# NVIDIA-AI-IOT/redtail

Hardware: AMD Instinct MI355X
Metric: stereo pairs/sec, ResNet18-2D 1257x369 (higher is better)
Workload: dtype f32

## Files before the change

### redtail_amd/csrc/kernels/conv_split.hip.h

```cpp
#pragma once
#include <type_traits>
#include "common.hip.h"
#include "conv_mfma.hip.h"

namespace rt {

constexpr float kSplitScale = 2048.f;
constexpr float kSplitInv = 1.f / 2048.f;

struct S3Split {
    f16x4 hi, lo;
};
__device__ static __forceinline__ S3Split s3_split(f32x4 v) {
    S3Split s;
#ifdef HIPEMU
#pragma unroll
    for (int j = 0; j < 4; j++) {
        const _Float16 h = (_Float16)v[j];
        s.hi[j] = h;
        s.lo[j] = (_Float16)((v[j] - (float)h) * kSplitScale);
    }
#else
    unsigned h[2], l[2];
#pragma unroll
// ... 198 lines not shown
        RT_TSTAMP();
    }
#ifdef RT_KERNEL_TIMING
    __builtin_amdgcn_s_waitcnt(0);
    if (dbgp && tid == 0) { dbgp[14] = __builtin_amdgcn_s_memtime(); dbgp[15] = __builtin_amdgcn_s_memrealtime() - rt0; }
#endif
}

}

namespace rt {

template <int KH, int KW, int S, int NW_ = 4>
struct S3Cfg {
    static constexpr int NW = NW_, TY = NW_, TX = 32, CC = 16, TAPS = KH * KW, NT = 64 * NW_;
    static constexpr int PR = (TY - 1) * S + KH, PC = (TX - 1) * S + KW;
    static constexpr int PCH = (PC + 1) / 2;
    static constexpr int PCL = S == 2 ? 2 * PCH : PC;
    static constexpr int NPART = NW / 4;
    static constexpr int NPIX = PR * PC, NKP = ((NPIX + NPART - 1) / NPART + 63) / 64;
    static constexpr int PXB = 80;
    static constexpr int W_SLOTS = TAPS * 2 * 2 * 32;
    static constexpr int NK_W = (W_SLOTS + NT - 1) / NT;
    static constexpr int IN_BYTES = PR * PCL * PXB, GRP_BYTES = IN_BYTES + W_SLOTS * 16;
    static constexpr int KS_MAX = NW_ != 4 ? 1 : (S == 2 ? 2 : 4);
    static constexpr int max_groups(int want) {
        int ks = want < 1 ? 1 : (want > KS_MAX ? KS_MAX : want);
        while (ks > 1 && (ks == 3 || ks * GRP_BYTES < (ks - 1) * NW * 64 * 16 * 4)) ks--;
        return ks;
    }
    static_assert(IN_BYTES % 16 == 0, "weight image alignment");
    static_assert(S == 1 || S == 2, "stride 1 or 2");
};

#ifndef RT_S3_WAVES
#define RT_S3_WAVES(S) ((S) == 2 ? 2 : 4)
#endif
template <int KH, int KW, int S, bool XIL, bool YIL, int NW = 4, typename TIN = float, typename TOUT = float>
__global__ void __launch_bounds__(64 * NW * (S3Cfg<KH, KW, S, NW>::KS_MAX)) RT_WAVES_PER_EU(RT_S3_WAVES(S)) conv_s3_kernel(ConvArgs p) {
    using Cfg = S3Cfg<KH, KW, S, NW>;
    constexpr bool XF16 = std::is_same<TIN, _Float16>::value, YF16 = std::is_same<TOUT, _Float16>::value;
    constexpr unsigned ESX = Io<TIN>::ES, ESY = Io<TOUT>::ES;
    static_assert(!XIL || !XF16, "interleaved fp16 input: conv_f16mma_kernel");
    constexpr int TY = Cfg::TY, TX = Cfg::TX, CC = Cfg::CC, TAPS = Cfg::TAPS, PC = Cfg::PC, PCL = Cfg::PCL, PXB = Cfg::PXB;
    constexpr int NKP = Cfg::NKP, NK_W = Cfg::NK_W, NT = Cfg::NT;

    constexpr int IN_BYTES = Cfg::IN_BYTES, GRP_BYTES = Cfg::GRP_BYTES;
#ifdef HIPEMU
    HIP_DYNAMIC_SHARED(char, smem)
#else
    extern __shared__ __attribute__((aligned(16))) char smem[];
#endif

    const int tid_wg = threadIdx.x;
    const int KS = Cfg::KS_MAX == 1 ? 1 : __builtin_amdgcn_readfirstlane((int)blockDim.x / NT);
    const int kgi = Cfg::KS_MAX == 1 ? 0 : __builtin_amdgcn_readfirstlane(tid_wg / NT);
    const int tid = tid_wg - kgi * NT;
    char* const sIn = smem + kgi * GRP_BYTES;
    f32x4* const sW = reinterpret_cast<f32x4*>(smem + kgi * GRP_BYTES + IN_BYTES);
#ifdef RT_KERNEL_TIMING
    unsigned long long* dbgp = (p.dbg && kgi == 0) ? p.dbg + ((size_t)(blockIdx.z * gridDim.y + blockIdx.y) * gridDim.x + blockIdx.x) * 16 : nullptr;
    int dbi = 0;
    const unsigned long long rt0 = __builtin_amdgcn_s_memrealtime();
#endif
    RT_TSTAMP();
    const int lane = tid & 63;
    const int kg = lane >> 5, l31 = lane & 31;
    const int wv = __builtin_amdgcn_readfirstlane(tid >> 6);

    RT_WG_TILE_NB(p, tile, zi, n, nblk)
    const int tx0 = (tile % p.tiles_x) * TX;
    const int ty0 = (tile / p.tiles_x) * TY;
    const char* __restrict__ xb = elem_ptr(p.x, (int64_t)n * p.x_bstride, ESX);
    const int nchunks = p.CinPad / CC;
    int pad_y = p.pad_y, pad_x = p.pad_x, Ho = p.Ho, Wo = p.Wo, ch_row = zi;
    int64_t y_off = p.y_off + (int64_t)zi * p.y_zstride, w_off = 0, r_off = y_off, r_off_il8 = y_off;
    int64_t y_off_il4 = 4 * p.y_off + (int64_t)zi * p.y_zstride, r_off_il4 = y_off_il4;
    unsigned tap_mask = ~0u;
    if (p.zs) {
        const ZSlice z = p.zs[zi];
        pad_y = z.pad_y; pad_x = z.pad_x; Ho = z.Ho; Wo = z.Wo; ch_row = z.ch_row; y_off = z.y_off; w_off = z.w_off;
        r_off = z.r_off; r_off_il8 = z.r_off_il8;
        y_off_il4 = 4 * z.y_off;
        r_off_il4 = z.r_off_il4;
        tap_mask = z.tap_mask;
    }
    const int act = p.act;

    const int sg = wv & 3, spart = wv >> 2;
    const int* __restrict__ tab = p.ch_off + (int64_t)ch_row * p.CinPad + 4 * sg;
    unsigned voff[NKP];
    int lidx[NKP], xcol[NKP];
    const int* __restrict__ shtab = p.ch_shift ? p.ch_shift + (int64_t)ch_row * p.CinPad + 4 * sg : nullptr;
#pragma unroll
    for (int k = 0; k < NKP; k++) {
        const int pidx = spart * (NKP * 64) + lane + 64 * k;
        const int pr = pidx / PC, pc = pidx - pr * PC;
        const int iy = ty0 * S - pad_y + pr, ix = tx0 * S - pad_x + pc;
        const bool own = pidx < Cfg::NPIX && lane + 64 * k < NKP * 64;
        xcol[k] = ix;
        voff[k] = (own && iy >= 0 && iy < p.Hi && ix >= 0 && ix < p.Wi) ? (unsigned)(iy * p.x_pitch + ix) * (XIL ? 16u : ESX) : kBufOOB;
        const int col = S == 2 ? (pc & 1) * Cfg::PCH + (pc >> 1) : pc;
        lidx[k] = own ? (pr * PCL + col) * PXB + sg * 8 : -1;
    }
    const char* __restrict__ wsrc = reinterpret_cast<const char*>(p.w) + (w_off + ((int64_t)nblk * nchunks) * Cfg::W_SLOTS) * 16;
    const buf_rsrc rs_w = make_buf(wsrc);

    f32x4 rin[NKP];
    f32x4 rw[NK_W];
    auto prefetch = [&](int ch) {
        if constexpr (XIL) {
            const int off = tab[ch * CC];
            const int sh = shtab ? shtab[ch * CC] : 0;
            const buf_rsrc rs = make_buf(xb, off >= 0);
#pragma unroll
            for (int k = 0; k < NKP; k++) {
                const unsigned vo = sh == 0 ? voff[k] : ((voff[k] != kBufOOB && xcol[k] >= sh) ? voff[k] - (unsigned)sh * 16u : kBufOOB);
                rin[k] = buf_load4(rs, vo, (unsigned)off * 4u);
            }
        } else {
            const int sh = shtab ? shtab[ch * CC] : 0;
#pragma unroll
            for (int j = 0; j < 4; j++) {
                const int off = tab[ch * CC + j];
                const buf_rsrc rs = make_buf(xb, off >= 0);
#pragma unroll
                for (int k = 0; k < NKP; k++) {
                    const unsigned vo = sh == 0 ? voff[k] : ((voff[k] != kBufOOB && xcol[k] >= sh) ? voff[k] - (unsigned)sh * ESX : kBufOOB);
                    rin[k][j] = Io<TIN>::load(rs, vo, (unsigned)off * ESX);
                }
            }
        }
        const unsigned so = (unsigned)ch * (unsigned)(Cfg::W_SLOTS * 16);
#pragma unroll
        for (int k = 0; k < NK_W; k++) {
            const int idx = tid + NT * k;
            rw[k] = buf_load4(rs_w, idx < Cfg::W_SLOTS ? (unsigned)idx * 16u : kBufOOB, so);
        }
    };
    auto stage_to_lds = [&]() {
#pragma unroll
        for (int k = 0; k < NKP; k++) {
            if (lidx[k] < 0) continue;
            if constexpr (XF16) {
                f16x4 h;
#pragma unroll
                for (int j = 0; j < 4; j++) h[j] = (_Float16)rin[k][j];
                *reinterpret_cast<f16x4*>(sIn + lidx[k]) = h;
            } else {
                const S3Split s = s3_split(rin[k]);
                *reinterpret_cast<f16x4*>(sIn + lidx[k]) = s.hi;
                *reinterpret_cast<f16x4*>(sIn + lidx[k] + 32) = s.lo;
            }
        }
#pragma unroll
        for (int k = 0; k < NK_W; k++) {
            const int idx = tid + NT * k;
            if (idx < Cfg::W_SLOTS) sW[idx] = rw[k];
        }
    };

    const int64_t ybase = (int64_t)n * p.y_bstride + y_off;
    const int64_t rbase = (int64_t)n * p.r_bstride + r_off;
    const int cs32 = (int)p.y_cstride, rs32 = (int)p.r_cstride;
    const int oy = ty0 + wv, ox = tx0 + l31;
    const bool inb = oy < Ho && ox < Wo;
    const bool r_il = p.r_il8 != 0;
    const int cb = nblk * 32;
    f32x4 rr[4];
    if (p.resid != nullptr && kgi == 0) {
        const buf_rsrc rs_r = make_buf(elem_ptr(p.resid, r_il ? (int64_t)n * p.r_bstride + (YF16 ? r_off_il8 : r_off_il4) : rbase, ESY));
        if (r_il && YF16) {
            const unsigned vo = inb ? (unsigned)((oy * p.y_ystride + ox * p.y_xstride) * 8 + 4 * kg) * 2u : kBufOOB;
#pragma unroll
            for (int q = 0; q < 4; q++) {
                const u32x2_t u = __builtin_amdgcn_raw_buffer_load_b64(rs_r, (cb + 8 * q + 4 * kg < p.Cout) ? vo : kBufOOB, (unsigned)((cb + 8 * q) * rs32) * 2u, 0);
#pragma unroll
                for (int e = 0; e < 4; e++) rr[q][e] = (float)__builtin_bit_cast(_Float16, (unsigned short)(u[e >> 1] >> (16 * (e & 1))));
            }
        } else if (r_il) {
            const unsigned vo = inb ? (unsigned)((oy * p.y_ystride + ox * p.y_xstride) * 4 + 4 * kg * rs32) * 4u : kBufOOB;
#pragma unroll
            for (int q = 0; q < 4; q++) rr[q] = buf_load4(rs_r, (cb + 8 * q + 4 * kg < p.Cout) ? vo : kBufOOB, (unsigned)((cb + 8 * q) * rs32) * 4u);
        } else {
            const unsigned vo = inb ? (unsigned)(oy * p.y_ystride + ox * p.y_xstride + 4 * kg * rs32) * ESY : kBufOOB;
#pragma unroll
            for (int q = 0; q < 4; q++)
#pragma unroll
                for (int e = 0; e < 4; e++)
                    rr[q][e] = Io<TOUT>::load(rs_r, (cb + 8 * q + 4 * kg + e < p.Cout) ? vo : kBufOOB, (unsigned)((cb + 8 * q + e) * rs32) * ESY);
        }
    } else {
#pragma unroll
        for (int q = 0; q < 4; q++) rr[q] = f32x4{0.f, 0.f, 0.f, 0.f};
    }

    f32x16 acc_m, acc_c;
#pragma unroll
    for (int r = 0; r < 16; r++) { acc_m[r] = 0.f; acc_c[r] = 0.f; }
    const int a_off = kg * 32 + l31;
    const bool w_exact = p.w_exact != 0;
    const int b_off = (wv * S * PCL + l31) * PXB + kg * 16;
    auto compute = [&]() {
#pragma unroll
        for (int t = 0; t < TAPS; t++) {
            if (!((tap_mask >> t) & 1u)) continue;
            const int r = t / KW, s = t % KW;
            const int col = S == 2 ? (s & 1) * Cfg::PCH + (s >> 1) : s;
            const char* bp = sIn + b_off + (r * PCL + col) * PXB;
            const f16x8 bh = *reinterpret_cast<const f16x8*>(bp);
            const f16x8 ah = __builtin_bit_cast(f16x8, sW[a_off + (t * 2 + 0) * 64]);
            acc_m = __builtin_amdgcn_mfma_f32_32x32x16_f16(ah, bh, acc_m, 0, 0, 0);
            if (!w_exact) {
                const f16x8 al = __builtin_bit_cast(f16x8, sW[a_off + (t * 2 + 1) * 64]);
                acc_c = __builtin_amdgcn_mfma_f32_32x32x16_f16(al, bh, acc_c, 0, 0, 0);
            }
            if constexpr (!XF16) {
                const f16x8 bl = *reinterpret_cast<const f16x8*>(bp + 32);
                acc_c = __builtin_amdgcn_mfma_f32_32x32x16_f16(ah, bl, acc_c, 0, 0, 0);
            }
        }
    };

    if (kgi < nchunks) prefetch(kgi);
    RT_TSTAMP();
    for (int ch = kgi; ch < nchunks + kgi; ch += KS) {
        const bool mine = KS == 1 || ch < nchunks;
        if (ch != kgi) __syncthreads();
        if (mine) stage_to_lds();
        __syncthreads();
        RT_TSTAMP();
        if (ch + KS < nchunks) prefetch(ch + KS);
        if (mine) compute();
        RT_TSTAMP();
    }

#pragma unroll
    for (int r = 0; r < 16; r++) acc_m[r] = fmaf(acc_c[r], kSplitInv, acc_m[r]);
    if (KS > 1) {
        f32x4* const red = reinterpret_cast<f32x4*>(smem);
        __syncthreads();
        if (kgi > 0) {
#pragma unroll
            for (int q = 0; q < 4; q++)
                red[(((kgi - 1) * NW + wv) * 4 + q) * 64 + lane] = f32x4{acc_m[4 * q], acc_m[4 * q + 1], acc_m[4 * q + 2], acc_m[4 * q + 3]};
        }
        __syncthreads();
        if (kgi > 0) return;
        for (int g = 1; g < KS; g++)
#pragma unroll
            for (int q = 0; q < 4; q++) {
                const f32x4 v = red[(((g - 1) * NW + wv) * 4 + q) * 64 + lane];
#pragma unroll
                for (int e = 0; e < 4; e++) acc_m[4 * q + e] += v[e];
            }
    }

    const buf_rsrc rs_y = make_buf(elem_ptr(p.y, (YIL && !YF16) ? (int64_t)n * p.y_bstride + y_off_il4 : ybase, ESY));
    auto epilogue = [&](auto ACT) {
#pragma unroll
        for (int q = 0; q < 4; q++) {
            const f32x4 bv = *reinterpret_cast<const f32x4*>(p.bias + cb + 8 * q + 4 * kg);
            f32x4 o;
#pragma unroll
            for (int e = 0; e < 4; e++)
                o[e] = apply_act_fast(acc_m[4 * q + e] + (bv[e] + rr[q][e]), decltype(ACT)::value);
            if constexpr (YIL && YF16) {
                const unsigned vo = (inb && cb + 8 * q + 4 * kg < p.Cout) ? (unsigned)((oy * p.y_ystride + ox * p.y_xstride) * 8 + 4 * kg) * 2u : kBufOOB;
                u32x2_t w2;
#pragma unroll
                for (int e = 0; e < 2; e++)
                    w2[e] = (unsigned)__builtin_bit_cast(unsigned short, (_Float16)o[2 * e]) | ((unsigned)__builtin_bit_cast(unsigned short, (_Float16)o[2 * e + 1]) << 16);
                __builtin_amdgcn_raw_buffer_store_b64(w2, rs_y, vo, (unsigned)((cb + 8 * q) * cs32) * 2u, 0);
            } else if constexpr (YIL) {
                const unsigned vo = (inb && cb + 8 * q + 4 * kg < p.Cout) ? (unsigned)((oy * p.y_ystride + ox * p.y_xstride) * 4 + 4 * kg * cs32) * 4u : kBufOOB;
                buf_store4(o, rs_y, vo, (unsigned)((cb + 8 * q) * cs32) * 4u);
            } else {
                const unsigned vo = inb ? (unsigned)(oy * p.y_ystride + ox * p.y_xstride + 4 * kg * cs32) * ESY : kBufOOB;
#pragma unroll
                for (int e = 0; e < 4; e++)
                    Io<TOUT>::store(o[e], rs_y, (cb + 8 * q + 4 * kg + e < p.Cout) ? vo : kBufOOB, (unsigned)((cb + 8 * q + e) * cs32) * ESY);
            }
        }
    };
    if (act == 1) epilogue(std::integral_constant<int, 1>{});
    else if (act == 2) epilogue(std::integral_constant<int, 2>{});
    else epilogue(std::integral_constant<int, 0>{});
    RT_TSTAMP();
#ifdef RT_KERNEL_TIMING
    __builtin_amdgcn_s_waitcnt(0);
    if (dbgp && tid == 0) { dbgp[14] = __builtin_amdgcn_s_memtime(); dbgp[15] = __builtin_amdgcn_s_memrealtime() - rt0; }
#endif
}

}

namespace rt {

struct S3FirstCfg {
    static constexpr int KH = 5, KW = 5, S = 2, TY = 4, TX = 32, CMAX = 3;
    static constexpr int PR = (TY - 1) * S + KH, PC = (TX - 1) * S + KW;
    static constexpr int NPAIR = (PC + 1) / 2;
    static constexpr int RS = 208;
    static constexpr int NTASK = CMAX * PR * NPAIR, NK = (NTASK + 255) / 256;
    static constexpr int W_SLOTS = KH * 2 * 2 * 32;
};

template <bool YIL>
__global__ void __launch_bounds__(256) RT_WAVES_PER_EU(4) conv_s3_first_kernel(ConvArgs p) {
    using Cfg = S3FirstCfg;
    constexpr int KH = Cfg::KH, S = Cfg::S, TY = Cfg::TY, TX = Cfg::TX, PR = Cfg::PR, NPAIR = Cfg::NPAIR, RS = Cfg::RS;

    __shared__ __attribute__((aligned(16))) _Float16 sHi[PR * RS];
    __shared__ __attribute__((aligned(16))) _Float16 sLo[PR * RS];

    const int tid = threadIdx.x;
    const int lane = tid & 63;
    const int kg = lane >> 5, l31 = lane & 31;
    const int wv = __builtin_amdgcn_readfirstlane(tid >> 6);

    int tile = blockIdx.x;
    if (p.xcd_order) {
        const int nwg = gridDim.x, q = nwg >> 3, r = nwg & 7;
        const int xcd = blockIdx.x & 7, idx = blockIdx.x >> 3;
        tile = (xcd < r ? xcd * (q + 1) : r * (q + 1) + (xcd - r) * q) + idx;
    }
    const int tx0 = (tile % p.tiles_x) * TX;
    const int ty0 = (tile / p.tiles_x) * TY;
    const int nblk = blockIdx.y;
    const int n = blockIdx.z;

    f32x4 wa[KH][2];
    {
        const buf_rsrc rs_w = make_buf(reinterpret_cast<const char*>(p.w) + (int64_t)nblk * Cfg::W_SLOTS * 16);
#pragma unroll
        for (int r = 0; r < KH; r++)
#pragma unroll
            for (int part = 0; part < 2; part++) wa[r][part] = buf_load4(rs_w, (unsigned)(((r * 2 + part) * 2 + kg) * 32 + l31) * 16u, 0);
    }

    const buf_rsrc rs_x = make_buf((p.x2 && n >= p.x2_from) ? p.x2 + (int64_t)(n - p.x2_from) * p.x_bstride : p.x + (int64_t)n * p.x_bstride);
    const int ix0 = tx0 * S - p.pad_x, iy0 = ty0 * S - p.pad_y;
    const int cin = p.cin_real;
#pragma unroll
    for (int k = 0; k < Cfg::NK; k++) {
        const int t = tid + 256 * k;
        const int c = t / (PR * NPAIR), rem = t - c * (PR * NPAIR);
        const int pr = rem / NPAIR, pc = 2 * (rem - pr * NPAIR);
        const int iy = iy0 + pr, ix = ix0 + pc;
        const bool own = t < Cfg::NTASK && c < cin;
        const bool row_ok = own && iy >= 0 && iy < p.Hi;
        const bool ok0 = row_ok && ix >= 0 && ix < p.Wi, ok1 = row_ok && ix + 1 >= 0 && ix + 1 < p.Wi && pc + 1 < Cfg::PC;
        const unsigned vo = (unsigned)((c * p.Hi + iy) * p.x_pitch + ix) * 4u;
        const float v0 = buf_load(rs_x, ok0 ? vo : kBufOOB, 0);
        const float v1 = buf_load(rs_x, ok1 ? vo + 4u : kBufOOB, 0);
        if (t < Cfg::NTASK) {
            const _Float16 h0 = (_Float16)v0, h1 = (_Float16)v1;
            const int o = pr * RS + pc * Cfg::CMAX + c;
            sHi[o] = h0;
            sHi[o + Cfg::CMAX] = h1;
            sLo[o] = (_Float16)((v0 - (float)h0) * kSplitScale);
            sLo[o + Cfg::CMAX] = (_Float16)((v1 - (float)h1) * kSplitScale);
        }
    }
    __syncthreads();

    f32x16 acc_m, acc_c;
#pragma unroll
    for (int r = 0; r < 16; r++) { acc_m[r] = 0.f; acc_c[r] = 0.f; }
    const unsigned* __restrict__ hi32 = reinterpret_cast<const unsigned*>(sHi);
    const unsigned* __restrict__ lo32 = reinterpret_cast<const unsigned*>(sLo);
#pragma unroll
    for (int r = 0; r < KH; r++) {
        const int base = ((wv * S + r) * RS + 6 * l31 + 8 * kg) >> 1;
        u32x4_t bh, bl;
#pragma unroll
        for (int e = 0; e < 4; e++) { bh[e] = hi32[base + e]; bl[e] = lo32[base + e]; }
        const f16x8 ah = __builtin_bit_cast(f16x8, wa[r][0]), al = __builtin_bit_cast(f16x8, wa[r][1]);
        acc_m = __builtin_amdgcn_mfma_f32_32x32x16_f16(ah, __builtin_bit_cast(f16x8, bh), acc_m, 0, 0, 0);
        acc_c = __builtin_amdgcn_mfma_f32_32x32x16_f16(al, __builtin_bit_cast(f16x8, bh), acc_c, 0, 0, 0);
        acc_c = __builtin_amdgcn_mfma_f32_32x32x16_f16(ah, __builtin_bit_cast(f16x8, bl), acc_c, 0, 0, 0);
    }

    const int oy = ty0 + wv, ox = tx0 + l31;
    const bool inb = oy < p.Ho && ox < p.Wo;
    const int cs32 = (int)p.y_cstride;
    const int cb = nblk * 32;
    const buf_rsrc rs_y = make_buf(elem_ptr(p.y, (int64_t)n * p.y_bstride + p.y_off, 4));
    const int act = p.act;
    auto epilogue = [&](auto ACT) {
#pragma unroll
        for (int q = 0; q < 4; q++) {
            const f32x4 bv = *reinterpret_cast<const f32x4*>(p.bias + cb + 8 * q + 4 * kg);
            f32x4 o;
#pragma unroll
            for (int e = 0; e < 4; e++) o[e] = apply_act_fast(fmaf(acc_c[4 * q + e], kSplitInv, acc_m[4 * q + e]) + bv[e], decltype(ACT)::value);
            if constexpr (YIL) {
                const unsigned vo = (inb && cb + 8 * q + 4 * kg < p.Cout) ? (unsigned)((oy * p.y_ystride + ox) * 4 + 4 * kg * cs32) * 4u : kBufOOB;
                buf_store4(o, rs_y, vo, (unsigned)((cb + 8 * q) * cs32) * 4u);
            } else {
                const unsigned vo = inb ? (unsigned)(oy * p.y_ystride + ox * p.y_xstride + 4 * kg * cs32) * 4u : kBufOOB;
#pragma unroll
                for (int e = 0; e < 4; e++)
                    buf_store(o[e], rs_y, (cb + 8 * q + 4 * kg + e < p.Cout) ? vo : kBufOOB, (unsigned)((cb + 8 * q + e) * cs32) * 4u);
            }
        }
    };
    if (act == 1) epilogue(std::integral_constant<int, 1>{});
    else if (act == 2) epilogue(std::integral_constant<int, 2>{});
    else epilogue(std::integral_constant<int, 0>{});
}

}

namespace rt {

struct S3RBCfg {
    static constexpr int NW = 4, TY = 4, TX = 32, NT = 256;
    static constexpr int XR = TY + 4, XC = TX + 4, XPIX = XR * XC;
    static constexpr int TR = TY + 2, TC = TX + 2, TPIX = TR * TC;
    static constexpr int TSEG = (TPIX + 31) / 32;
    static constexpr int SEGW = (TSEG + NW - 1) / NW;
    static constexpr int PXB = 80;
    static constexpr int NSLOT = XPIX * 4, NKX = (NSLOT + NT - 1) / NT;
    static constexpr int W_SLOTS = 9 * 2 * 2 * 32, NK_W = (W_SLOTS + NT - 1) / NT;
};

struct RBArgs {
    ConvArgs c;
    const float* w1;
    const float* bias1;
    int act1;
    int cmid;
    int seg;
};

template <bool XIL, bool YIL>
__global__ void __launch_bounds__(256) RT_WAVES_PER_EU(2) conv_s3rb_kernel(RBArgs a) {
    using Cfg = S3RBCfg;
    const ConvArgs& p = a.c;
    constexpr int TY = Cfg::TY, TX = Cfg::TX, XC = Cfg::XC, TC = Cfg::TC, PXB = Cfg::PXB, NT = Cfg::NT;
    constexpr int NKX = Cfg::NKX, NK_W = Cfg::NK_W, SEGW = Cfg::SEGW;

    __shared__ __attribute__((aligned(16))) f32x4 sW[Cfg::W_SLOTS];
    __shared__ __attribute__((aligned(16))) char sX[Cfg::XPIX * PXB];
    __shared__ __attribute__((aligned(16))) char sT[2][Cfg::TSEG * 32 * PXB];

    const int tid = threadIdx.x;
#ifdef RT_KERNEL_TIMING
    unsigned long long* dbgp = p.dbg ? p.dbg + ((size_t)blockIdx.z * gridDim.x + blockIdx.x) * 16 : nullptr;
    int dbi = 0;
    const unsigned long long rt0 = __builtin_amdgcn_s_memrealtime();
#endif
    RT_TSTAMP();
    const int lane = tid & 63;
    const int kg = lane >> 5, l31 = lane & 31;
    const int wv = __builtin_amdgcn_readfirstlane(tid >> 6);

    int tile = blockIdx.x;
    if (p.xcd_order) {
        const int nwg = gridDim.x, q = nwg >> 3, r = nwg & 7;
        const int xcd = blockIdx.x & 7, idx = blockIdx.x >> 3;
        tile = (xcd < r ? xcd * (q + 1) : r * (q + 1) + (xcd - r) * q) + idx;
    }
    const int tx0 = (tile % p.tiles_x) * TX;
    const int ty0 = (tile / p.tiles_x) * TY;
    const int n = blockIdx.z;
    const int H = p.Hi, W = p.Wi;

    const buf_rsrc rs_x = make_buf(elem_ptr(p.x, (int64_t)n * p.x_bstride, 4));
    const unsigned cs_x = (unsigned)p.x_cstride;
    unsigned xoff[NKX];
    int xg[NKX], xlds[NKX];
#pragma unroll
    for (int k = 0; k < NKX; k++) {
        const int idx = tid + NT * k;
        const int g = idx / Cfg::XPIX, pix = idx - g * Cfg::XPIX;
        const int pr = pix / XC, pc = pix - pr * XC;
        const int iy = ty0 - 2 + pr, ix = tx0 - 2 + pc;
        const bool in = idx < Cfg::NSLOT && iy >= 0 && iy < H && ix >= 0 && ix < W;
        xoff[k] = in ? (unsigned)(iy * p.x_pitch + ix) * (XIL ? 16u : 4u) : kBufOOB;
        xg[k] = g;
        xlds[k] = idx < Cfg::NSLOT ? pix * PXB + g * 8 : -1;
    }
    f32x4 rin[NKX];
    f32x4 rw[NK_W];
    auto gather_x = [&](int ch) {
#pragma unroll
        for (int k = 0; k < NKX; k++) {
            const int c0 = 16 * ch + 4 * xg[k];
            const bool ok = xoff[k] != kBufOOB && c0 < p.cin_real;
            if constexpr (XIL) {
                rin[k] = buf_load4(rs_x, ok ? (unsigned)c0 * cs_x * 4u + xoff[k] : kBufOOB, 0u);
            } else {
#pragma unroll
                for (int j = 0; j < 4; j++)
                    rin[k][j] = buf_load(rs_x, (ok && c0 + j < p.cin_real) ? (unsigned)(c0 + j) * cs_x * 4u + xoff[k] : kBufOOB, 0u);
            }
        }
    };
    auto gather_w = [&](const float* w, int ch) {
        const buf_rsrc rs_w = make_buf(w);
#pragma unroll
        for (int k = 0; k < NK_W; k++) {
            const int idx = tid + NT * k;
            rw[k] = buf_load4(rs_w, idx < Cfg::W_SLOTS ? (unsigned)idx * 16u : kBufOOB, (unsigned)ch * (unsigned)(Cfg::W_SLOTS * 16));
        }
    };
    auto stage_x = [&]() {
#pragma unroll
        for (int k = 0; k < NKX; k++) {
            if (xlds[k] < 0) continue;
            const S3Split s = s3_split(rin[k]);
            *reinterpret_cast<f16x4*>(sX + xlds[k]) = s.hi;
            *reinterpret_cast<f16x4*>(sX + xlds[k] + 32) = s.lo;
        }
    };
    auto stage_w = [&]() {
#pragma unroll
        for (int k = 0; k < NK_W; k++) {
            const int idx = tid + NT * k;
            if (idx < Cfg::W_SLOTS) sW[idx] = rw[k];
        }
    };
    const int a_off = kg * 32 + l31;
    auto contract = [&](const char* bp0, int row_pitch, f32x16& acc_m, f32x16& acc_c) {
#pragma unroll
        for (int t = 0; t < 9; t++) {
            const int r = t / 3, s = t % 3;
            const char* bp = bp0 + (r * row_pitch + s) * PXB;
            const f16x8 bh = *reinterpret_cast<const f16x8*>(bp);
            const f16x8 bl = *reinterpret_cast<const f16x8*>(bp + 32);
            const f16x8 ah = __builtin_bit_cast(f16x8, sW[a_off + (t * 2 + 0) * 64]);
            const f16x8 al = __builtin_bit_cast(f16x8, sW[a_off + (t * 2 + 1) * 64]);
            acc_m = __builtin_amdgcn_mfma_f32_32x32x16_f16(ah, bh, acc_m, 0, 0, 0);
            acc_c = __builtin_amdgcn_mfma_f32_32x32x16_f16(al, bh, acc_c, 0, 0, 0);
            acc_c = __builtin_amdgcn_mfma_f32_32x32x16_f16(ah, bl, acc_c, 0, 0, 0);
        }
    };

    int pt[SEGW], bx[SEGW];
#pragma unroll
    for (int i = 0; i < SEGW; i++) {
        pt[i] = (wv + Cfg::NW * i) * 32 + l31;
        const int tr = pt[i] / TC, tc = pt[i] - tr * TC;
        bx[i] = (pt[i] < Cfg::TPIX ? (tr * XC + tc) * PXB : 0) + kg * 16;
    }
    f32x16 am[SEGW], ac[SEGW];
#pragma unroll
    for (int i = 0; i < SEGW; i++)
#pragma unroll
        for (int r = 0; r < 16; r++) { am[i][r] = 0.f; ac[i][r] = 0.f; }
    const bool seg1 = wv + Cfg::NW < Cfg::TSEG;

    gather_x(0);
    gather_w(a.w1, 0);
    RT_TSTAMP();
#pragma unroll
    for (int ch = 0; ch < 2; ch++) {
        if (ch) __syncthreads();
        stage_x();
        stage_w();
        __syncthreads();
        RT_TSTAMP();
        if (ch == 0) { gather_x(1); gather_w(a.w1, 1); }
        else gather_w(p.w, 0);
        contract(sX + bx[0], XC, am[0], ac[0]);
        if (seg1) contract(sX + bx[1], XC, am[1], ac[1]);
        RT_TSTAMP();
    }
#pragma unroll
    for (int i = 0; i < SEGW; i++) {
        if (i == 1 && !seg1) break;
        if (pt[i] < Cfg::TPIX) {
            const int tr = pt[i] / TC, tc = pt[i] - tr * TC;
            const int gy = ty0 - 1 + tr, gx = tx0 - 1 + tc;
            const bool inside = gy >= 0 && gy < H && gx >= 0 && gx < W;
#pragma unroll
            for (int q = 0; q < 4; q++) {
                const f32x4 bv = *reinterpret_cast<const f32x4*>(a.bias1 + 8 * q + 4 * kg);
                f32x4 o;
#pragma unroll
                for (int e = 0; e < 4; e++) {
                    const float v = apply_act_fast(fmaf(ac[i][4 * q + e], kSplitInv, am[i][4 * q + e]) + bv[e], a.act1);
                    o[e] = (inside && 8 * q + 4 * kg + e < a.cmid) ? v : 0.f;
                }
                const S3Split s = s3_split(o);
                char* dst = sT[q >> 1] + pt[i] * PXB + (8 * (q & 1) + 4 * kg) * 2;
                *reinterpret_cast<f16x4*>(dst) = s.hi;
                *reinterpret_cast<f16x4*>(dst + 32) = s.lo;
            }
        }
    }
    RT_TSTAMP();

    const int oy = ty0 + wv, ox = tx0 + l31;
    const bool inb = oy < p.Ho && ox < p.Wo;
    const int cs32 = (int)p.y_cstride, rs32 = (int)p.r_cstride;
    f32x4 rr[4];
    {
        const buf_rsrc rs_r = make_buf(elem_ptr(p.resid, (int64_t)n * p.r_bstride, 4), p.resid != nullptr);
        if (p.r_il8) {
            const unsigned vo = inb ? (unsigned)((oy * p.x_pitch + ox) * 4 + 4 * kg * rs32) * 4u : kBufOOB;
#pragma unroll
            for (int q = 0; q < 4; q++) rr[q] = buf_load4(rs_r, (8 * q + 4 * kg < p.Cout) ? vo : kBufOOB, (unsigned)(8 * q * rs32) * 4u);
        } else {
            const unsigned vo = inb ? (unsigned)(oy * p.x_pitch + ox + 4 * kg * rs32) * 4u : kBufOOB;
#pragma unroll
            for (int q = 0; q < 4; q++)
#pragma unroll
                for (int e = 0; e < 4; e++)
                    rr[q][e] = buf_load(rs_r, (8 * q + 4 * kg + e < p.Cout) ? vo : kBufOOB, (unsigned)((8 * q + e) * rs32) * 4u);
        }
    }
    f32x16 acc_m, acc_c;
#pragma unroll
    for (int r = 0; r < 16; r++) { acc_m[r] = 0.f; acc_c[r] = 0.f; }
    const int b2 = (wv * TC + l31) * PXB + kg * 16;
#pragma unroll
    for (int ch = 0; ch < 2; ch++) {
        __syncthreads();
        stage_w();
        __syncthreads();
        if (ch == 0) gather_w(p.w, 1);
        contract(sT[ch] + b2, TC, acc_m, acc_c);
        RT_TSTAMP();
    }
    const buf_rsrc rs_y = make_buf(elem_ptr(p.y, (int64_t)n * p.y_bstride + p.y_off, 4));
    const int act = p.act;
    auto epilogue = [&](auto ACT) {
#pragma unroll
        for (int q = 0; q < 4; q++) {
            const f32x4 bv = *reinterpret_cast<const f32x4*>(p.bias + 8 * q + 4 * kg);
            f32x4 o;
#pragma unroll
            for (int e = 0; e < 4; e++)
                o[e] = apply_act_fast(fmaf(acc_c[4 * q + e], kSplitInv, acc_m[4 * q + e]) + (bv[e] + rr[q][e]), decltype(ACT)::value);
            if constexpr (YIL) {
                const unsigned vo = (inb && 8 * q + 4 * kg < p.Cout) ? (unsigned)((oy * p.y_ystride + ox) * 4 + 4 * kg * cs32) * 4u : kBufOOB;
                buf_store4(o, rs_y, vo, (unsigned)(8 * q * cs32) * 4u);
            } else {
                const unsigned vo = inb ? (unsigned)(oy * p.y_ystride + ox * p.y_xstride + 4 * kg * cs32) * 4u : kBufOOB;
#pragma unroll
                for (int e = 0; e < 4; e++)
                    buf_store(o[e], rs_y, (8 * q + 4 * kg + e < p.Cout) ? vo : kBufOOB, (unsigned)((8 * q + e) * cs32) * 4u);
            }
        }
    };
    if (act == 1) epilogue(std::integral_constant<int, 1>{});
    else if (act == 2) epilogue(std::integral_constant<int, 2>{});
    else epilogue(std::integral_constant<int, 0>{});
    RT_TSTAMP();
#ifdef RT_KERNEL_TIMING
    __builtin_amdgcn_s_waitcnt(0);
    if (dbgp && tid == 0) { dbgp[14] = __builtin_amdgcn_s_memtime(); dbgp[15] = __builtin_amdgcn_s_memrealtime() - rt0; }
#endif
}

}
```

### redtail_amd/csrc/kernels/deconv3d_small.hip.h

```cpp
#pragma once
#include "common.hip.h"
#include "conv_split.hip.h"

namespace rt {

struct Deconv3dSmallArgs {
    const float* x;
    float* y;
    const float* w;
    const float* bias;
    const float* resid;
    int K, Dy, Hy, Wy;
    int Dx, Hx, Wx, C;
    int bz, by, bx;
    int Mz;
    int xp, yp;
    int act;
    int64_t x_bstride, y_bstride;
    int sparse;
};

template <bool Z, int PAT = 0>
struct SmallTaps {
    static constexpr int NJ = Z ? 8 : 4, ND = Z ? 3 : 2;
    static constexpr bool valid(int f, int j) {
        for (int d = 0; d < ND; d++) {
            const int fd = (f >> d) & 1, jd = (j >> d) & 1;
            if ((PAT >> d) & 1) { if (fd == 1 && jd == 0) return false; }
            else if (fd == 0 && jd == 1) return false;
        }
        return true;
    }
    static constexpr int index(int f, int j) {
        int n = 0;
        for (int ff = 0; ff < NJ; ff++)
            for (int jj = 0; jj < NJ; jj++) {
                if (ff == f && jj == j) return n;
                n += valid(ff, jj) ? 1 : 0;
            }
        return n;
    }
    static constexpr int NV = Z ? 27 : 9;
};

template <int COUT, bool Z = true, typename TIN = float, typename TOUT = float>
__global__ void __launch_bounds__(256) deconv3d_s2_small_kernel(Deconv3dSmallArgs p) {
    constexpr int NJ = Z ? 8 : 4;
    constexpr unsigned ESX = Io<TIN>::ES, ESY = Io<TOUT>::ES;
    const int mx = blockIdx.x * 256 + threadIdx.x;
    const int my = blockIdx.y;
    const int mz = blockIdx.z % p.Mz, n = blockIdx.z / p.Mz;

    unsigned voff[NJ];
#pragma unroll
    for (int j = 0; j < NJ; j++) {
        const int iz = Z ? mz + p.bz + (j >> 2) : 0, iy = my + p.by + ((j >> 1) & 1), ix = mx + p.bx + (j & 1);
        const bool ok = iz >= 0 && iz < p.Dy && iy >= 0 && iy < p.Hy && ix >= 0 && ix < p.Wy;
        voff[j] = ok ? (unsigned)((iz * p.Hy + iy) * p.xp + ix) * ESX : kBufOOB;
    }
    const buf_rsrc rs_x = make_buf(elem_ptr(p.x, (int64_t)n * p.x_bstride, ESX));
    const unsigned cstride = (unsigned)(p.Dy * p.Hy * p.xp) * ESX;

    float acc[COUT][NJ];
#pragma unroll
    for (int co = 0; co < COUT; co++)
#pragma unroll
        for (int f = 0; f < NJ; f++) acc[co][f] = p.bias[co];

    const float* __restrict__ wk = p.w;
    auto contract_sparse = [&](auto taps) {
        using Taps = decltype(taps);
        for (int k = 0; k < p.K; k++, wk += COUT * Taps::NV) {
            float xv[NJ];
#pragma unroll
            for (int j = 0; j < NJ; j++) xv[j] = Io<TIN>::load(rs_x, voff[j], (unsigned)k * cstride);
#pragma unroll
            for (int co = 0; co < COUT; co++)
#pragma unroll
                for (int f = 0; f < NJ; f++)
#pragma unroll
                    for (int j = 0; j < NJ; j++)
                        if (Taps::valid(f, j)) acc[co][f] = fmaf(xv[j], wk[co * Taps::NV + Taps::index(f, j)], acc[co][f]);
        }
    };
    if (p.sparse == 1) contract_sparse(SmallTaps<Z, 0>{});
    else if (Z && p.sparse == 1 + 4) contract_sparse(SmallTaps<Z, Z ? 4 : 0>{});
    else {
        for (int k = 0; k < p.K; k++, wk += COUT * NJ * NJ) {
            float xv[NJ];
#pragma unroll
            for (int j = 0; j < NJ; j++) xv[j] = Io<TIN>::load(rs_x, voff[j], (unsigned)k * cstride);
#pragma unroll
            for (int co = 0; co < COUT; co++)
#pragma unroll
                for (int f = 0; f < NJ; f++)
#pragma unroll
                    for (int j = 0; j < NJ; j++) acc[co][f] = fmaf(xv[j], wk[(co * NJ + f) * NJ + j], acc[co][f]);
        }
    }

    const buf_rsrc rs_y = make_buf(elem_ptr(p.y, (int64_t)n * p.y_bstride, ESY));
    const buf_rsrc rs_r = make_buf(elem_ptr(p.resid, (int64_t)n * p.y_bstride, ESY), p.resid != nullptr);
    const int ox = 2 * mx;
#pragma unroll
    for (int co = 0; co < COUT; co++) {
        if (co >= p.C) break;
#pragma unroll
        for (int pz = 0; pz < (Z ? 2 : 1); pz++)
#pragma unroll
            for (int py = 0; py < 2; py++) {
                const int oz = Z ? 2 * mz + pz : 0, oy = 2 * my + py;
                const bool row_ok = oz < p.Dx && oy < p.Hx;
                const unsigned off = (unsigned)(((oz * p.C + co) * p.Hx + oy) * p.yp + ox) * ESY;
                const unsigned v2 = (row_ok && ox + 1 < p.Wx) ? off : kBufOOB;
                const unsigned v1 = (row_ok && ox + 1 == p.Wx) ? off : kBufOOB;
                f32x2_t o = {acc[co][4 * pz + 2 * py], acc[co][4 * pz + 2 * py + 1]};
                const f32x2_t r2 = Io<TOUT>::load2(rs_r, v2, 0);
                const float r1 = Io<TOUT>::load(rs_r, v1, 0);
                o[0] = apply_act_rt(o[0] + r2[0] + r1, p.act);
                o[1] = apply_act_rt(o[1] + r2[1], p.act);
                Io<TOUT>::store2(o, rs_y, v2, 0);
                Io<TOUT>::store(o[0], rs_y, v1, 0);
            }
    }
}

constexpr int kSmallIlIters = 3;
constexpr float kSaLog2e = 1.44269504088896341f;
typedef _Float16 f16x8_small __attribute__((ext_vector_type(8)));

__global__ void __launch_bounds__(256) deconv3d_s2_il_kernel(Deconv3dSmallArgs p) {
    const int tid = threadIdx.x, lane = tid & 63, n16 = lane & 15, q = lane >> 4;
    const int wv = __builtin_amdgcn_readfirstlane(tid >> 6);
    int lin = blockIdx.x;
    {
        const int nwg = gridDim.x, q_ = nwg >> 3, r_ = nwg & 7, xcd = blockIdx.x & 7, idx = blockIdx.x >> 3;
        lin = (xcd < r_ ? xcd * (q_ + 1) : r_ * (q_ + 1) + (xcd - r_) * q_) + idx;
    }
    const int mz = lin % p.Mz, bx = lin / p.Mz;
    const int my0 = 2 * blockIdx.y, n = blockIdx.z;
    const int KC = p.K / 32;
    const int ngroups = (int)cdiv((p.Wx + 1) / 2, 16);
    const buf_rsrc rs_x = make_buf(elem_ptr(p.x, (int64_t)n * p.x_bstride, 2));
    const buf_rsrc rs_w = make_buf(p.w);
    const buf_rsrc rs_y = make_buf(elem_ptr(p.y, (int64_t)n * p.y_bstride, 4));
    const buf_rsrc rs_r = make_buf(elem_ptr(p.resid, (int64_t)n * p.y_bstride, 4), p.resid != nullptr);
    const unsigned gstride = (unsigned)(p.Dy * p.Hy * p.xp) * 16u;
    const int co = q >> 1, fz = q & 1;
    const float bias = co < p.C ? p.bias[co] : 0.f;
    const bool has_r = p.resid != nullptr;
    const int nrows = (p.Hx + 1) / 2;

    f32x4 a0[8];
    if (KC == 1) {
#pragma unroll
        for (int j = 0; j < 8; j++) a0[j] = buf_load4(rs_w, (unsigned)(j * 64 + lane) * 16u, 0);
    }
    for (int it = 0; it < kSmallIlIters; it++) {
        const int grp = (bx * 4 + wv) * kSmallIlIters + it;
        if (grp >= ngroups) break;
        const int mx = grp * 16 + n16;
        f32x4 acc[2] = {{bias, bias, bias, bias}, {bias, bias, bias, bias}};
        for (int kc = 0; kc < KC; kc++) {
            f32x4 b[2][3][2];
#pragma unroll
            for (int jz = 0; jz < 2; jz++)
#pragma unroll
                for (int ry = 0; ry < 3; ry++)
#pragma unroll
                    for (int jx = 0; jx < 2; jx++) {
                        const int iz = mz + p.bz + jz, iy = my0 + p.by + ry, ix = mx + p.bx + jx;
                        const bool ok = iz >= 0 && iz < p.Dy && iy >= 0 && iy < p.Hy && ix >= 0 && ix < p.Wy;
                        const unsigned vo = ok ? (unsigned)((iz * p.Hy + iy) * p.xp + ix) * 16u + (unsigned)(kc * 4 + q) * gstride : kBufOOB;
                        b[jz][ry][jx] = buf_load4(rs_x, vo, 0);
                    }
#pragma unroll
            for (int j = 0; j < 8; j++) {
                const f32x4 av = KC == 1 ? a0[j] : buf_load4(rs_w, (unsigned)((j * KC + kc) * 64 + lane) * 16u, 0);
                const f16x8_small a = __builtin_bit_cast(f16x8_small, av);
#pragma unroll
                for (int row = 0; row < 2; row++)
                    acc[row] = __builtin_amdgcn_mfma_f32_16x16x32_f16(a, __builtin_bit_cast(f16x8_small, b[j >> 2][row + ((j >> 1) & 1)][j & 1]), acc[row], 0, 0, 0);
            }
        }
        const int oz = 2 * mz + fz, ox = 2 * mx;
#pragma unroll
        for (int row = 0; row < 2; row++) {
            if (my0 + row >= nrows) break;
#pragma unroll
            for (int fy = 0; fy < 2; fy++) {
                const int oy = 2 * (my0 + row) + fy;
                const bool row_ok = co < p.C && oz < p.Dx && oy < p.Hx;
                const unsigned off = (unsigned)(((oz * p.C + co) * p.Hx + oy) * p.yp + ox) * 4u;
                const unsigned v2 = (row_ok && ox + 1 < p.Wx) ? off : kBufOOB;
                const unsigned v1 = (row_ok && ox + 1 == p.Wx) ? off : kBufOOB;
                f32x2_t o = {acc[row][2 * fy], acc[row][2 * fy + 1]};
                if (has_r) {
                    const f32x2_t r2 = buf_load2(rs_r, v2, 0);
                    const float r1 = buf_load(rs_r, v1, 0);
                    o[0] += r2[0] + r1;
                    o[1] += r2[1];
                }
                o[0] = apply_act_rt(o[0], p.act);
                o[1] = apply_act_rt(o[1], p.act);
                buf_store2(o, rs_y, v2, 0);
                buf_store(o[0], rs_y, v1, 0);
            }
        }
    }
}

template <int SA>
__global__ void __launch_bounds__(256) RT_WAVES_PER_EU(3) deconv3d_s2_ilw_kernel(Deconv3dSmallArgs p, int seg_len, int nseg) {
    const int tid = threadIdx.x, lane = tid & 63, n16 = lane & 15, q = lane >> 4;
    const int wv = __builtin_amdgcn_readfirstlane(tid >> 6);
    const int seg = blockIdx.x % nseg, bxg = blockIdx.x / nseg;
    const int my0 = 2 * blockIdx.y, n = blockIdx.z;
    const int ngroups = (int)cdiv((p.Wx + 1) / 2, 16);
    const int grp = bxg * 4 + wv;
    if (grp >= ngroups) return;
    const int z0 = seg * seg_len, z1 = z0 + seg_len < p.Mz ? z0 + seg_len : p.Mz;
    const buf_rsrc rs_x = make_buf(elem_ptr(p.x, (int64_t)n * p.x_bstride, 2));
    const buf_rsrc rs_w = make_buf(p.w);
    const buf_rsrc rs_y = make_buf(elem_ptr(p.y, (int64_t)n * p.y_bstride, 4));
    const buf_rsrc rs_r = make_buf(elem_ptr(p.resid, (int64_t)n * p.y_bstride, 4), p.resid != nullptr);
    const unsigned gstride = (unsigned)(p.Dy * p.Hy * p.xp) * 16u;
    const int co = q >> 1, fz = q & 1;
    const float bias = co < p.C ? p.bias[co] : 0.f;
    const bool has_r = p.resid != nullptr;
    const int nrows = (p.Hx + 1) / 2;
    const int mx = grp * 16 + n16;

    f32x4 a0[8];
#pragma unroll
    for (int j = 0; j < 8; j++) a0[j] = buf_load4(rs_w, (unsigned)(j * 64 + lane) * 16u, 0);

    unsigned pos[3][2];
#pragma unroll
    for (int ry = 0; ry < 3; ry++)
#pragma unroll
        for (int jx = 0; jx < 2; jx++) {
            const int iy = my0 + p.by + ry, ix = mx + p.bx + jx;
            pos[ry][jx] = (iy >= 0 && iy < p.Hy && ix >= 0 && ix < p.Wy) ? (unsigned)(iy * p.xp + ix) * 16u + (unsigned)q * gstride : kBufOOB;
        }
    const unsigned zbytes = (unsigned)(p.Hy * p.xp) * 16u;
    auto load_slice = [&](f32x4 (&b)[3][2], int iz) __attribute__((always_inline)) {
        const bool ok = iz >= 0 && iz < p.Dy;
#pragma unroll
        for (int ry = 0; ry < 3; ry++)
#pragma unroll
            for (int jx = 0; jx < 2; jx++) b[ry][jx] = buf_load4(rs_x, ok ? pos[ry][jx] : kBufOOB, ok ? (unsigned)iz * zbytes : 0u);
    };
    float sa_m[2][4], sa_s[2][4], sa_w[2][4];
#pragma unroll
    for (int row = 0; row < 2; row++)
#pragma unroll
        for (int j = 0; j < 4; j++) { sa_m[row][j] = -1e30f; sa_s[row][j] = 0.f; sa_w[row][j] = 0.f; }
    auto block = [&](int mz, const f32x4 (&b0)[3][2], const f32x4 (&b1)[3][2]) __attribute__((always_inline)) {
        f32x4 acc[2] = {{bias, bias, bias, bias}, {bias, bias, bias, bias}};
#pragma unroll
        for (int j = 0; j < 8; j++) {
            const f16x8_small a = __builtin_bit_cast(f16x8_small, a0[j]);
#pragma unroll
            for (int row = 0; row < 2; row++) {
                const f32x4 bv = (j >> 2) ? b1[row + ((j >> 1) & 1)][j & 1] : b0[row + ((j >> 1) & 1)][j & 1];
                acc[row] = __builtin_amdgcn_mfma_f32_16x16x32_f16(a, __builtin_bit_cast(f16x8_small, bv), acc[row], 0, 0, 0);
            }
        }
        const int oz = 2 * mz + fz, ox = 2 * mx;
        if constexpr (SA != 0) {
            const bool z_ok = oz < p.Dx;
            const float fzv = (float)oz;
            if (p.act != 0) {
#pragma unroll
                for (int row = 0; row < 2; row++)
#pragma unroll
                    for (int j = 0; j < 4; j++) acc[row][j] = apply_act_rt(acc[row][j], p.act);
            }
#pragma unroll
            for (int row = 0; row < 2; row++)
#pragma unroll
                for (int j = 0; j < 4; j++) {
                    const float v = acc[row][j] * (SA == 2 ? -kSaLog2e : kSaLog2e);
                    const float xv = z_ok ? v : -INFINITY;
                    const float mn = fmaxf(sa_m[row][j], xv);
                    const float c = __builtin_amdgcn_exp2f(sa_m[row][j] - mn), e = __builtin_amdgcn_exp2f(xv - mn);
                    sa_s[row][j] = sa_s[row][j] * c + e;
                    sa_w[row][j] = sa_w[row][j] * c + e * fzv;
                    sa_m[row][j] = mn;
                }
        } else {
#pragma unroll
            for (int row = 0; row < 2; row++) {
                if (my0 + row >= nrows) break;
#pragma unroll
                for (int fy = 0; fy < 2; fy++) {
                    const int oy = 2 * (my0 + row) + fy;
                    const bool row_ok = co < p.C && oz < p.Dx && oy < p.Hx;
                    const unsigned off = (unsigned)(((oz * p.C + co) * p.Hx + oy) * p.yp + ox) * 4u;
                    const unsigned v2 = (row_ok && ox + 1 < p.Wx) ? off : kBufOOB;
                    const unsigned v1 = (row_ok && ox + 1 == p.Wx) ? off : kBufOOB;
                    f32x2_t o = {acc[row][2 * fy], acc[row][2 * fy + 1]};
                    if (has_r) {
                        const f32x2_t r2 = buf_load2(rs_r, v2, 0);
                        const float r1 = buf_load(rs_r, v1, 0);
                        o[0] += r2[0] + r1;
                        o[1] += r2[1];
                    }
                    if (p.act != 0) {
                        o[0] = apply_act_rt(o[0], p.act);
                        o[1] = apply_act_rt(o[1], p.act);
                    }
                    buf_store2(o, rs_y, v2, 0);
                    buf_store(o[0], rs_y, v1, 0);
                }
            }
        }
    };

    f32x4 s0[3][2], s1[3][2], s2[3][2];
    load_slice(s0, z0 + p.bz);
    load_slice(s1, z0 + p.bz + 1);
    for (int mz = z0; mz < z1; mz += 3) {
        load_slice(s2, mz + p.bz + 2);
        block(mz, s0, s1);
        if (mz + 1 >= z1) break;
        load_slice(s0, mz + p.bz + 3);
        block(mz + 1, s1, s2);
        if (mz + 2 >= z1) break;
        load_slice(s1, mz + p.bz + 4);
        block(mz + 2, s2, s0);
    }
    if constexpr (SA != 0) {
        const int ox = 2 * mx;
#pragma unroll
        for (int row = 0; row < 2; row++)
#pragma unroll
            for (int j = 0; j < 4; j++) {
                const float m1 = __shfl_xor(sa_m[row][j], 16), s1v = __shfl_xor(sa_s[row][j], 16), w1v = __shfl_xor(sa_w[row][j], 16);
                const float mn = fmaxf(sa_m[row][j], m1);
                const float c0 = __builtin_amdgcn_exp2f(sa_m[row][j] - mn), c1 = __builtin_amdgcn_exp2f(m1 - mn);
                const float st = sa_s[row][j] * c0 + s1v * c1, wt = sa_w[row][j] * c0 + w1v * c1;
                const int oy = 2 * (my0 + row) + (j >> 1), oxj = ox + (j & 1);
                const bool ok = q == 0 && oy < p.Hx && oxj < p.Wx;
                buf_store(wt / st, rs_y, ok ? (unsigned)(oy * p.Wx + oxj) * 4u : kBufOOB, 0);
            }
    }
}

__global__ void __launch_bounds__(256) deconv3d_s2_il4_kernel(Deconv3dSmallArgs p) {
    const int tid = threadIdx.x, lane = tid & 63, n16 = lane & 15, q = lane >> 4;
    const int wv = __builtin_amdgcn_readfirstlane(tid >> 6);
    int lin = blockIdx.x;
    {
        const int nwg = gridDim.x, q_ = nwg >> 3, r_ = nwg & 7, xcd = blockIdx.x & 7, idx = blockIdx.x >> 3;
        lin = (xcd < r_ ? xcd * (q_ + 1) : r_ * (q_ + 1) + (xcd - r_) * q_) + idx;
    }
    const int mz = lin % p.Mz, bx = lin / p.Mz;
    const int my0 = 2 * blockIdx.y, n = blockIdx.z;
    const int KC = p.K / 32;
    const int ngroups = (int)cdiv((p.Wx + 1) / 2, 16);
    const buf_rsrc rs_x = make_buf(elem_ptr(p.x, (int64_t)n * p.x_bstride, 4));
    const buf_rsrc rs_w = make_buf(p.w);
    const buf_rsrc rs_y = make_buf(elem_ptr(p.y, (int64_t)n * p.y_bstride, 4));
    const buf_rsrc rs_r = make_buf(elem_ptr(p.resid, (int64_t)n * p.y_bstride, 4), p.resid != nullptr);
    const unsigned gstride = (unsigned)(p.Dy * p.Hy * p.xp) * 16u;
    const int co = q >> 1, fz = q & 1;
    const float bias = co < p.C ? p.bias[co] : 0.f;
    const bool has_r = p.resid != nullptr;
    const int nrows = (p.Hx + 1) / 2;

    f32x4 ah0[8], al0[8];
    if (KC == 1) {
#pragma unroll
        for (int j = 0; j < 8; j++) {
            ah0[j] = buf_load4(rs_w, (unsigned)(j * 64 + lane) * 16u, 0);
            al0[j] = buf_load4(rs_w, (unsigned)((8 + j) * 64 + lane) * 16u, 0);
        }
    }
    for (int it = 0; it < kSmallIlIters; it++) {
        const int grp = (bx * 4 + wv) * kSmallIlIters + it;
        if (grp >= ngroups) break;
        const int mx = grp * 16 + n16;
        f32x4 acc_m[2] = {{bias, bias, bias, bias}, {bias, bias, bias, bias}};
        f32x4 acc_c[2] = {{0.f, 0.f, 0.f, 0.f}, {0.f, 0.f, 0.f, 0.f}};
        for (int kc = 0; kc < KC; kc++) {
#pragma unroll
            for (int jz = 0; jz < 2; jz++) {
// ... 61 lines not shown
```

Measured before the change: 2684.

## Vectorize first-conv input gather and share deconv neighbor loads via DPP

In the first strided conv, each lane now gathers a run of four pixels for all three channels with 16-byte loads and writes packed 8-byte LDS stores, replacing per-element scalar loads and 2-byte LDS writes. The bias is loaded early instead of inside the epilogue. In the 2D sparse small deconv, each lane loads only the even-column inputs and gets the right neighbor through a DPP lane shift. The wave-edge value comes from a separate load broadcast with readlane, and loads are grouped in channel blocks with double buffering. This cuts global load count and adds software pipelining, at the cost of more registers and more complex boundary handling.

```diff
diff --git a/redtail_amd/csrc/kernels/conv_split.hip.h b/redtail_amd/csrc/kernels/conv_split.hip.h
--- a/redtail_amd/csrc/kernels/conv_split.hip.h
+++ b/redtail_amd/csrc/kernels/conv_split.hip.h
@@ -524,14 +524,15 @@
     static constexpr int PR = (TY - 1) * S + KH, PC = (TX - 1) * S + KW;
     static constexpr int NPAIR = (PC + 1) / 2;
     static constexpr int RS = 208;
-    static constexpr int NTASK = CMAX * PR * NPAIR, NK = (NTASK + 255) / 256;
+    static constexpr int NRUN = NPAIR / 2, NRUN_T = PR * NRUN;
+    static_assert(NPAIR % 2 == 0 && NRUN_T <= 256 && (RS * 2) % 8 == 0 && NRUN * 4 * CMAX <= RS, "one gather per lane, 8-byte LDS writes");
     static constexpr int W_SLOTS = KH * 2 * 2 * 32;
 };
 
 template <bool YIL>
 __global__ void __launch_bounds__(256) RT_WAVES_PER_EU(4) conv_s3_first_kernel(ConvArgs p) {
     using Cfg = S3FirstCfg;
-    constexpr int KH = Cfg::KH, S = Cfg::S, TY = Cfg::TY, TX = Cfg::TX, PR = Cfg::PR, NPAIR = Cfg::NPAIR, RS = Cfg::RS;
+    constexpr int KH = Cfg::KH, S = Cfg::S, TY = Cfg::TY, TX = Cfg::TX, PR = Cfg::PR, RS = Cfg::RS;
 
     __shared__ __attribute__((aligned(16))) _Float16 sHi[PR * RS];
     __shared__ __attribute__((aligned(16))) _Float16 sLo[PR * RS];
@@ -561,28 +562,49 @@
             for (int part = 0; part < 2; part++) wa[r][part] = buf_load4(rs_w, (unsigned)(((r * 2 + part) * 2 + kg) * 32 + l31) * 16u, 0);
     }
 
+    const int cb = nblk * 32;
+    f32x4 bv[4];
+#pragma unroll
+    for (int q = 0; q < 4; q++) bv[q] = *reinterpret_cast<const f32x4*>(p.bias + cb + 8 * q + 4 * kg);
+
     const buf_rsrc rs_x = make_buf((p.x2 && n >= p.x2_from) ? p.x2 + (int64_t)(n - p.x2_from) * p.x_bstride : p.x + (int64_t)n * p.x_bstride);
     const int ix0 = tx0 * S - p.pad_x, iy0 = ty0 * S - p.pad_y;
     const int cin = p.cin_real;
-#pragma unroll
-    for (int k = 0; k < Cfg::NK; k++) {
-        const int t = tid + 256 * k;
-        const int c = t / (PR * NPAIR), rem = t - c * (PR * NPAIR);
-        const int pr = rem / NPAIR, pc = 2 * (rem - pr * NPAIR);
+    if (tid < Cfg::NRUN_T) {
+        const int pr = (int)((unsigned)tid / (unsigned)Cfg::NRUN), pc = 4 * (tid - pr * Cfg::NRUN);
         const int iy = iy0 + pr, ix = ix0 + pc;
-        const bool own = t < Cfg::NTASK && c < cin;
-        const bool row_ok = own && iy >= 0 && iy < p.Hi;
-        const bool ok0 = row_ok && ix >= 0 && ix < p.Wi, ok1 = row_ok && ix + 1 >= 0 && ix + 1 < p.Wi && pc + 1 < Cfg::PC;
-        const unsigned vo = (unsigned)((c * p.Hi + iy) * p.x_pitch + ix) * 4u;
-        const float v0 = buf_load(rs_x, ok0 ? vo : kBufOOB, 0);
-        const float v1 = buf_load(rs_x, ok1 ? vo + 4u : kBufOOB, 0);
-        if (t < Cfg::NTASK) {
-            const _Float16 h0 = (_Float16)v0, h1 = (_Float16)v1;
-            const int o = pr * RS + pc * Cfg::CMAX + c;
-            sHi[o] = h0;
-            sHi[o + Cfg::CMAX] = h1;
-            sLo[o] = (_Float16)((v0 - (float)h0) * kSplitScale);
-            sLo[o + Cfg::CMAX] = (_Float16)((v1 - (float)h1) * kSplitScale);
+        const bool row_ok = iy >= 0 && iy < p.Hi;
+        const bool whole = row_ok && ix >= 0 && ix + 3 < p.Wi;
+        const unsigned vo = (unsigned)(iy * p.x_pitch + ix) * 4u, cs = (unsigned)(p.Hi * p.x_pitch) * 4u;
+        f32x4 v[Cfg::CMAX];
+#pragma unroll
+        for (int c = 0; c < Cfg::CMAX; c++) v[c] = buf_load4(rs_x, (whole && c < cin) ? vo + c * cs : kBufOOB, 0);
+        if (row_ok && !whole) {
+#pragma unroll
+            for (int c = 0; c < Cfg::CMAX; c++)
+#pragma unroll
+                for (int e = 0; e < 4; e++)
+                    v[c][e] = buf_load(rs_x, (c < cin && ix + e >= 0 && ix + e < p.Wi) ? vo + c * cs + 4u * e : kBufOOB, 0);
+        }
+        if (pc + 3 >= Cfg::PC) {
+#pragma unroll
+            for (int c = 0; c < Cfg::CMAX; c++) v[c][3] = 0.f;
+        }
+        unsigned short hh[4 * Cfg::CMAX], ll[4 * Cfg::CMAX];
+#pragma unroll
+        for (int e = 0; e < 4; e++)
+#pragma unroll
+            for (int c = 0; c < Cfg::CMAX; c++) {
+                const _Float16 h = (_Float16)v[c][e];
+                hh[e * Cfg::CMAX + c] = __builtin_bit_cast(unsigned short, h);
+                ll[e * Cfg::CMAX + c] = __builtin_bit_cast(unsigned short, (_Float16)((v[c][e] - (float)h) * kSplitScale));
+            }
+        u32x2_t* const dh = reinterpret_cast<u32x2_t*>(sHi + pr * RS + pc * Cfg::CMAX);
+        u32x2_t* const dl = reinterpret_cast<u32x2_t*>(sLo + pr * RS + pc * Cfg::CMAX);
+#pragma unroll
+        for (int i = 0; i < 3; i++) {
+            dh[i] = u32x2_t{(unsigned)hh[4 * i] | ((unsigned)hh[4 * i + 1] << 16), (unsigned)hh[4 * i + 2] | ((unsigned)hh[4 * i + 3] << 16)};
+            dl[i] = u32x2_t{(unsigned)ll[4 * i] | ((unsigned)ll[4 * i + 1] << 16), (unsigned)ll[4 * i + 2] | ((unsigned)ll[4 * i + 3] << 16)};
         }
     }
     __syncthreads();
@@ -607,16 +629,14 @@
     const int oy = ty0 + wv, ox = tx0 + l31;
     const bool inb = oy < p.Ho && ox < p.Wo;
     const int cs32 = (int)p.y_cstride;
-    const int cb = nblk * 32;
     const buf_rsrc rs_y = make_buf(elem_ptr(p.y, (int64_t)n * p.y_bstride + p.y_off, 4));
     const int act = p.act;
     auto epilogue = [&](auto ACT) {
 #pragma unroll
         for (int q = 0; q < 4; q++) {
-            const f32x4 bv = *reinterpret_cast<const f32x4*>(p.bias + cb + 8 * q + 4 * kg);
             f32x4 o;
 #pragma unroll
-            for (int e = 0; e < 4; e++) o[e] = apply_act_fast(fmaf(acc_c[4 * q + e], kSplitInv, acc_m[4 * q + e]) + bv[e], decltype(ACT)::value);
+            for (int e = 0; e < 4; e++) o[e] = apply_act_fast(fmaf(acc_c[4 * q + e], kSplitInv, acc_m[4 * q + e]) + bv[q][e], decltype(ACT)::value);
             if constexpr (YIL) {
                 const unsigned vo = (inb && cb + 8 * q + 4 * kg < p.Cout) ? (unsigned)((oy * p.y_ystride + ox) * 4 + 4 * kg * cs32) * 4u : kBufOOB;
                 buf_store4(o, rs_y, vo, (unsigned)((cb + 8 * q) * cs32) * 4u);
diff --git a/redtail_amd/csrc/kernels/deconv3d_small.hip.h b/redtail_amd/csrc/kernels/deconv3d_small.hip.h
--- a/redtail_amd/csrc/kernels/deconv3d_small.hip.h
+++ b/redtail_amd/csrc/kernels/deconv3d_small.hip.h
@@ -43,6 +43,25 @@
     static constexpr int NV = Z ? 27 : 9;
 };
 
+constexpr int kSmallU = 8;
+
+__device__ static __forceinline__ float lane_right(float v, float last) {
+#ifdef HIPEMU
+    const float r = __shfl_down(v, 1);
+    return (threadIdx.x & 63) == 63 ? last : r;
+#else
+    return __builtin_bit_cast(float, __builtin_amdgcn_update_dpp(__builtin_bit_cast(int, last), __builtin_bit_cast(int, v), 0x130, 0xf, 0xf, false));
+#endif
+}
+__device__ static __forceinline__ int lane_get(int v, int l) {
+#ifdef HIPEMU
+    return __shfl(v, l);
+#else
+    return __builtin_amdgcn_readlane(v, l);
+#endif
+}
+__device__ static __forceinline__ float lane_get(float v, int l) { return __builtin_bit_cast(float, lane_get(__builtin_bit_cast(int, v), l)); }
+
 template <int COUT, bool Z = true, typename TIN = float, typename TOUT = float>
 __global__ void __launch_bounds__(256) deconv3d_s2_small_kernel(Deconv3dSmallArgs p) {
     constexpr int NJ = Z ? 8 : 4;
@@ -83,7 +102,57 @@
                         if (Taps::valid(f, j)) acc[co][f] = fmaf(xv[j], wk[co * Taps::NV + Taps::index(f, j)], acc[co][f]);
         }
     };
-    if (p.sparse == 1) contract_sparse(SmallTaps<Z, 0>{});
+    auto contract_sparse_2d = [&]() {
+        using Taps = SmallTaps<false, 0>;
+        constexpr int U = kSmallU;
+        const int lane = threadIdx.x & 63;
+        const unsigned e0 = (unsigned)lane_get((int)voff[1], 63), e1 = (unsigned)lane_get((int)voff[3], 63);
+        const unsigned veoff = (lane < U ? e0 : (lane < 2 * U ? e1 : kBufOOB)) + (unsigned)(lane % U) * cstride;
+        auto load_group = [&](float (&xo)[U][2], float& xe, int k0) __attribute__((always_inline)) {
+#pragma unroll
+            for (int u = 0; u < U; u++)
+#pragma unroll
+                for (int jy = 0; jy < 2; jy++) xo[u][jy] = Io<TIN>::load(rs_x, voff[2 * jy], (unsigned)(k0 + u) * cstride);
+            xe = Io<TIN>::load(rs_x, veoff, (unsigned)k0 * cstride);
+        };
+        auto channel = [&](const float (&xo)[2], float xe, int u) __attribute__((always_inline)) {
+            const float xv[4] = {xo[0], lane_right(xo[0], lane_get(xe, u)), xo[1], lane_right(xo[1], lane_get(xe, U + u))};
+#pragma unroll
+            for (int co = 0; co < COUT; co++)
+#pragma unroll
+                for (int f = 0; f < 4; f++)
+#pragma unroll
+                    for (int j = 0; j < 4; j++)
+                        if (Taps::valid(f, j)) acc[co][f] = fmaf(xv[j], wk[co * Taps::NV + Taps::index(f, j)], acc[co][f]);
+            wk += COUT * Taps::NV;
+        };
+        auto group = [&](const float (&xo)[U][2], float xe) __attribute__((always_inline)) {
+#pragma unroll
+            for (int u = 0; u < U; u++) channel(xo[u], xe, u);
+        };
+        const int ng = p.K / U;
+        float xo0[U][2], xo1[U][2], xe0, xe1;
+        if (ng > 0) load_group(xo0, xe0, 0);
+        for (int g = 0; g < ng; g += 2) {
+            if (g + 1 < ng) load_group(xo1, xe1, (g + 1) * U);
+            group(xo0, xe0);
+            if (g + 1 >= ng) break;
+            if (g + 2 < ng) load_group(xo0, xe0, (g + 2) * U);
+            group(xo1, xe1);
+        }
+        const int rem = p.K - ng * U;
+        if (rem > 0) {
+            const float xe = Io<TIN>::load(rs_x, lane % U < rem ? veoff : kBufOOB, (unsigned)(ng * U) * cstride);
+            for (int u = 0; u < rem; u++) {
+                float xo[2];
+#pragma unroll
+                for (int jy = 0; jy < 2; jy++) xo[jy] = Io<TIN>::load(rs_x, voff[2 * jy], (unsigned)(ng * U + u) * cstride);
+                channel(xo, xe, u);
+            }
+        }
+    };
+    if (!Z && p.sparse == 1) { if constexpr (!Z) contract_sparse_2d(); }
+    else if (p.sparse == 1) contract_sparse(SmallTaps<Z, 0>{});
     else if (Z && p.sparse == 1 + 4) contract_sparse(SmallTaps<Z, Z ? 4 : 0>{});
     else {
         for (int k = 0; k < p.K; k++, wk += COUT * NJ * NJ) {
```

Result: faster. 2722, median of 6 (+1.4%).
